# f-dangel/vivit

Measured on AMD Instinct MI355X. Metric: GGN eigenpairs/sec (Gram build + symeig), MLP 784-512-10, batch=4096, higher is better.
Workload: dtype f32

## Files before the change

### vivit_amd/csrc/common.h

```cpp
#pragma once
#include <hip/hip_runtime.h>
#include <stddef.h>
#include <stdint.h>

#include "../../include/vivit_hip.h"

namespace vivit {

typedef float f32x16 __attribute__((ext_vector_type(16)));
typedef float f32x4 __attribute__((ext_vector_type(4)));

static inline int64_t cdiv(int64_t a, int64_t b) { return (a + b - 1) / b; }
static inline size_t align_up(size_t x, size_t a) { return (x + a - 1) / a * a; }

static inline int launch_status() {
  return hipGetLastError() == hipSuccess ? VIVIT_OK : VIVIT_E_LAUNCH;
}

static inline bool ensure_dynamic_lds(const void *fn, int bytes, unsigned long long &done) {
  int dev = 0;
  if (hipGetDevice(&dev) != hipSuccess) return false;
  const unsigned long long bit = 1ull << (dev & 63);
  if (done & bit) return true;
  if (hipFuncSetAttribute(fn, hipFuncAttributeMaxDynamicSharedMemorySize, bytes) != hipSuccess) return false;
  return true;
}

enum { LAY_K = 0, LAY_M = 1 };

struct GemmDesc {
  const float *A;
  const float *B;
  float *C;
  int64_t M, N, K, lda, ldb, ldc;
};

struct GemmArgs {
  const float *A;
  const float *B;
  float *C;
  int64_t M, N, K, lda, ldb, ldc;
  float alpha, beta;
  int ksplit;
  int64_t kchunk;
  float *slab;
  int tiles_m, tiles_n;
  int syrk;
  int a_vec, b_vec;
  const GemmDesc *desc;
  int sbw;
  const int *gate = nullptr;
  int gate_mask = 0;
};

int gemm_launch(int alay, int blay, const float *A, const float *B, float *C, int64_t M, int64_t N,
                int64_t K, int64_t lda, int64_t ldb, int64_t ldc, float alpha, float beta, bool syrk,
                void *workspace, size_t workspace_bytes, hipStream_t stream);
size_t gemm_workspace_bytes(int64_t M, int64_t N, int64_t K, bool syrk);
int gemm_lower_launch(const float *A, const float *B, float *C, int64_t n, int64_t K, int64_t lda, int64_t ldb,
                      int64_t ldc, float alpha, float beta, hipStream_t stream);
int gemm_batched_launch(int alay, int blay, const GemmDesc *desc, int batch, int64_t maxM, int64_t maxN, float alpha,
                        float beta, hipStream_t stream);

bool skinny_applicable(int64_t M, int64_t N, int64_t K);
size_t skinny_workspace_bytes(int64_t K, int64_t n, int64_t P);
int skinny_nn_launch(const float *coef, int64_t ldc_, const float *V, int64_t ldv, float *out, int64_t ldo, int64_t K,
                     int64_t n, int64_t P, float alpha, float beta, void *ws, size_t ws_bytes, hipStream_t stream);

bool prof_enabled();
int prof_stride();
void prof_begin(int kind, double work, hipStream_t stream);
void prof_end(int kind, hipStream_t stream);
enum { PROF_STAGE_BEGIN = 0, PROF_STAGE_PREP = 1, PROF_STAGE_SY2SB = 2, PROF_STAGE_SB2ST = 3, PROF_STAGE_TRIDIAG = 4,
       PROF_STAGE_Q2 = 5, PROF_STAGE_Q1 = 6, PROF_STAGE_OUTPUT = 7, PROF_STAGE_SYTRD = 8,
       PROF_STAGE_SY2SB_PP = 9, PROF_STAGE_SY2SB_UPD = 10, PROF_NUM_STAGES = 11 };
void prof_mark(int stage, hipStream_t stream);

int *persist_timeout_word(hipStream_t stream);
int persist_override();
int persist_fault();

inline int device_cu_count() {
  static int cached[64] = {0};
  int dev = 0;
  if (hipGetDevice(&dev) != hipSuccess) return 0;
  int &c = cached[dev & 63];
  if (c == 0) {
    int v = 0;
    if (hipDeviceGetAttribute(&v, hipDeviceAttributeMultiprocessorCount, dev) != hipSuccess) v = -1;
    c = v > 0 ? v : -1;
  }
  return c;
}

}
```

### vivit_amd/csrc/gemm64.hip

```cpp
#include "gemm_plan.h"

namespace vivit {

constexpr int G64_NST = 7;
constexpr int G64_TA = 64 * BK, G64_TB = 256 * BK, G64_STG = G64_TA + G64_TB;
constexpr int GEMM64_LDS_BYTES = G64_NST * G64_STG * 4;

template <int ALAY, int BLAY>
__global__ __launch_bounds__(256, 1) void gemm64_dma_kernel(GemmArgs p) {
  extern __shared__ __attribute__((aligned(16))) float smem3[];
  if (p.gate && (*p.gate & p.gate_mask) == 0) return;
  const int tj = blockIdx.x;
  const int tid = threadIdx.x, lane = tid & 63, wave = tid >> 6;
  const int r = lane & 31, h = lane >> 5;
  const int64_t col0 = (int64_t)tj * 256;
  const int64_t kbeg = (int64_t)blockIdx.y * p.kchunk;
  const int64_t kend = (kbeg + p.kchunk < p.K) ? kbeg + p.kchunk : p.K;
  const int nt = (int)((kend - kbeg) / BK);

  f32x16 acc[2][2];
  auto clear_acc = [&]() __attribute__((always_inline)) {
#pragma unroll
    for (int i = 0; i < 2; ++i)
#pragma unroll
// ... 324 lines not shown
static bool gemm64_attrs() {
  static unsigned long long attr_done = 0;
  int dev = 0;
  if (hipGetDevice(&dev) != hipSuccess) return false;
  if (attr_done & (1ull << (dev & 63))) return true;
  const struct { const void *fn; int bytes; } kernels[] = {
      {reinterpret_cast<const void *>(gemm64_dma_kernel<LAY_K, LAY_K>), GEMM64_LDS_BYTES},
      {reinterpret_cast<const void *>(gemm64_dma_kernel<LAY_K, LAY_M>), GEMM64_LDS_BYTES},
      {reinterpret_cast<const void *>(gemm64_dma_kernel<LAY_M, LAY_K>), GEMM64_LDS_BYTES},
      {reinterpret_cast<const void *>(gemm64_dma_kernel<LAY_M, LAY_M>), GEMM64_LDS_BYTES},
      {reinterpret_cast<const void *>(gemm64_bx_kernel<LAY_K>), GEMM64X_LDS_BYTES},
      {reinterpret_cast<const void *>(gemm64_bx_kernel<LAY_M>), GEMM64X_LDS_BYTES},
      {reinterpret_cast<const void *>(gemm64_bx_kernel<LAY_K, true>), GEMM64X_LDS_BYTES},
      {reinterpret_cast<const void *>(gemm64_bx_kernel<LAY_M, true>), GEMM64X_LDS_BYTES}};
  for (const auto &k : kernels)
    if (!ensure_dynamic_lds(k.fn, k.bytes, attr_done)) return false;
  attr_done |= 1ull << (dev & 63);
  return true;
}

bool plan_gemm64(const GemmShape &sh, GemmPlan &pl) {
  const int64_t M = sh.M, N = sh.N, K = sh.K;
  if (sh.syrk || !(M <= 64 && N >= 2048 && K >= 2048 && (K % BK) == 0)) return false;
  pl = GemmPlan{};
  pl.route = GemmRoute::Gemm64;
  const int64_t tiles = cdiv(N, 256), ktiles = K / BK;
  int64_t s = 1;
  double best = 0.0;
  for (int64_t c = 1; c <= 24; ++c) {
    if (c > 1 && ktiles / c < 64) break;
    const int64_t wgs = tiles * c;
    const double fill = (double)wgs / (double)(256 * cdiv(wgs, 256));
    const double score = wgs >= 512 ? fill : fill * 0.5 * (double)wgs / 512.0;
    if (score > best + 1e-9) { best = score; s = c; }
  }
  pl.kchunk = cdiv(ktiles, s) * BK;
  pl.ksplit = (int)cdiv(K, pl.kchunk);
  const bool strict = gemm64_bx_enabled() && sh.pub;
  pl.slab_bytes = (pl.ksplit > 1 || strict) ? (size_t)pl.ksplit * (size_t)M * (size_t)N * sizeof(float) : 0;
  pl.bytes = pl.slab_bytes;
  if (!gemm64_bx_enabled()) return true;
  pl.a_off = align_up(pl.slab_bytes, 256);
  const size_t pieces_end = pl.a_off + (size_t)ktiles * 6144;
  pl.flags_off = align_up(pieces_end, 256);
  pl.bytes = strict ? pl.flags_off + 256 : pieces_end;
  return true;
}

static bool gemm64_bx_reach(int blay, int64_t ldb) {
  return (int64_t)(blay == LAY_K ? 255 : 15) * ldb * 4 + 1024 < ((int64_t)1 << 32);
}

int launch_gemm64(const GemmPlan &pl, const GemmShape &sh, int alay, int blay, GemmArgs p, void *workspace, size_t workspace_bytes,
                         hipStream_t stream) {
  p.ksplit = pl.ksplit;
  p.kchunk = pl.kchunk;
  const bool bx = gemm64_bx_enabled() && gemm64_bx_reach(blay, p.ldb);
  const bool strict = bx && sh.pub;
  p.slab = nullptr;
  if (p.ksplit > 1 || strict) {
    if (!workspace || workspace_bytes < pl.slab_bytes) return VIVIT_E_WORKSPACE;
    p.slab = ws_at<float>(workspace, pl.slab_off);
  }
  uint4 *apieces = nullptr;
  int *flag = nullptr;
  if (bx) {
    if (!workspace || workspace_bytes < pl.bytes) return VIVIT_E_WORKSPACE;
    apieces = ws_at<uint4>(workspace, pl.a_off);
    if (strict) flag = ws_at<int>(workspace, pl.flags_off);
  }
  if (!gemm64_attrs()) return VIVIT_E_LAUNCH;
  if (flag && hipMemsetAsync(flag, 0, sizeof(int), stream) != hipSuccess) return VIVIT_E_LAUNCH;
  p.tiles_m = 1;
  p.tiles_n = (int)cdiv(p.N, 256);
  p.syrk = 0;
  p.desc = nullptr;
  dim3 grid((unsigned)p.tiles_n, (unsigned)p.ksplit, 1);
  auto launch_dma = [&](const GemmArgs &q) {
    with_layouts(alay, blay, [&](auto LA, auto LB) { gemm64_dma_kernel<LA, LB><<<grid, 256, GEMM64_LDS_BYTES, stream>>>(q); });
  };
  const unsigned kt = (unsigned)(p.K / BK);
  if (strict) {
    with_layout(alay, [&](auto L) { g64_split_a_kernel<L, true><<<kt, 128, 0, stream>>>(p.A, p.lda, p.M, apieces, flag); });
    with_layout(blay, [&](auto L) { gemm64_bx_kernel<L, true><<<grid, 256, GEMM64X_LDS_BYTES, stream>>>(p, apieces, flag); });
    int st = launch_status();
    if (st != VIVIT_OK) return st;
    GemmArgs f = p;
    f.gate = flag;
    f.gate_mask = tls_bx_gate_mask;
    launch_dma(f);
  } else if (bx) {
    with_layout(alay, [&](auto L) { g64_split_a_kernel<L><<<kt, 128, 0, stream>>>(p.A, p.lda, p.M, apieces, nullptr); });
    with_layout(blay, [&](auto L) { gemm64_bx_kernel<L><<<grid, 256, GEMM64X_LDS_BYTES, stream>>>(p, apieces, nullptr); });
  } else {
    launch_dma(p);
  }
  int st = launch_status();
  if (st != VIVIT_OK) return st;
  if (p.slab) {
    launch_gemm_reduce(p.slab, p.C, p.M, p.N, p.ldc, p.ksplit, p.alpha, p.beta, 0, stream);
    st = launch_status();
  }
  return st;
}

}
```

### vivit_amd/csrc/gemm_f32.hip

```cpp
#include "gemm_plan.h"

namespace vivit {

__global__ __launch_bounds__(256) void gemm_reduce_kernel(const float *__restrict__ slab, float *__restrict__ C,
                                                          int64_t M, int64_t N, int64_t ldc, int ksplit,
                                                          float alpha, float beta, int syrk, int tile = BM) {
  const int64_t idx = (int64_t)blockIdx.x * 256 + threadIdx.x;
  if (idx >= M * N) return;
  const int64_t i = idx / N, j = idx - i * N;
  int64_t src = idx;
  if (syrk && (j / tile) > (i / tile)) src = j * N + i;
  float s = 0.f;
  for (int z = 0; z < ksplit; ++z) s += slab[(int64_t)z * M * N + src];
  float v = alpha * s;
  if (beta != 0.f) v += beta * C[i * ldc + j];
  C[i * ldc + j] = v;
}
void launch_gemm_reduce(const float *slab, float *C, int64_t M, int64_t N, int64_t ldc, int ksplit, float alpha, float beta, int syrk,
                        hipStream_t stream, int tile) {
  gemm_reduce_kernel<<<(unsigned)cdiv(M * N, 256), 256, 0, stream>>>(slab, C, M, N, ldc, ksplit, alpha, beta, syrk, tile);
}

__global__ __launch_bounds__(256) void scale_c_kernel(float *__restrict__ C, int64_t M, int64_t N, int64_t ldc, float beta) {
  const int64_t idx = (int64_t)blockIdx.x * 256 + threadIdx.x;
  if (idx >= M * N) return;
  const int64_t i = idx / N, j = idx - i * N;
  C[i * ldc + j] = beta == 0.f ? 0.f : beta * C[i * ldc + j];
}
void launch_scale_c(float *C, int64_t M, int64_t N, int64_t ldc, float beta, hipStream_t stream) {
  scale_c_kernel<<<(unsigned)cdiv(M * N, 256), 256, 0, stream>>>(C, M, N, ldc, beta);
}

size_t gemm_workspace_bytes(int64_t M, int64_t N, int64_t K, bool syrk) {
  if (M <= 0 || N <= 0 || K <= 0) return 0;
  const GemmShape sh{M, N, K, syrk, syrk, bx_public_product()};
  GemmShape whole = sh;
  whole.K = K / BK * BK;
  size_t b = 0;
  GemmPlan pl;
  if (plan_tile256_bx(whole, pl) && pl.bytes > b) b = pl.bytes;
  if (plan_tile256(whole, pl) && pl.bytes > b) b = pl.bytes;
  if (plan_bx_splitk(whole, pl) && pl.bytes > b) b = pl.bytes;
  if (plan_gemm64(whole, pl) && pl.bytes > b) b = pl.bytes;
  if (plan_tsk(sh, pl) && pl.bytes > b) b = pl.bytes;
  if (plan_tile128(sh, pl) && pl.bytes > b) b = pl.bytes;
  return b;
}

int gemm_launch(int alay, int blay, const float *A, const float *B, float *C, int64_t M, int64_t N,
                int64_t K, int64_t lda, int64_t ldb, int64_t ldc, float alpha, float beta, bool syrk,
                void *workspace, size_t workspace_bytes, hipStream_t stream) {
  if (M < 0 || N < 0 || K < 0) return VIVIT_E_BADARG;
  if (M == 0 || N == 0) return VIVIT_OK;
  if (!C || ldc < N) return VIVIT_E_BADARG;
  if (K == 0) {
    launch_scale_c(C, M, N, ldc, beta, stream);
    return launch_status();
  }
  if (!A || !B) return VIVIT_E_BADARG;
  if (lda < (alay == LAY_K ? K : M) || ldb < (blay == LAY_K ? K : N)) return VIVIT_E_BADARG;
  if (syrk && (M != N || alay != blay)) return VIVIT_E_BADARG;

  GemmArgs p;
  p.A = A; p.B = B; p.C = C;
  p.M = M; p.N = N; p.K = K; p.lda = lda; p.ldb = ldb; p.ldc = ldc;
  p.alpha = alpha; p.beta = beta;
  const GemmShape sh{M, N, K, syrk, A == B && lda == ldb && M == N && alay == blay, bx_public_product()};
  const bool ptr_vec = operand_vec(A, lda) && operand_vec(B, ldb);
  const auto holds = [&](const GemmPlan &q) { return workspace && workspace_bytes >= q.bytes; };
  GemmPlan pl;
  if (ptr_vec && (alay == LAY_K || (M & 3) == 0) && (blay == LAY_K || (N & 3) == 0)) {
    GemmShape whole = sh;
    whole.K = p.K = K / BK * BK;
    bool on256 = true;
    int st = VIVIT_OK;
    if (plan_tile256_bx(whole, pl) && holds(pl)) {
      st = launch_tile256_bx(pl, whole, alay, blay, p, workspace, stream);
    } else if (plan_tile256(whole, pl)) {
      if (pl.ksplit > 1 && !holds(pl)) {
        const size_t fit = workspace ? workspace_bytes / ((size_t)M * (size_t)N * sizeof(float)) : 1;
        plan_tile256(whole, pl, fit < 1 ? 1 : (int)(fit < 4 ? fit : 4));
      }
      st = launch_tile256(pl, whole, alay, blay, p, workspace, stream);
    } else if (plan_bx_splitk(whole, pl) && holds(pl)) {
      st = launch_bx_splitk(pl, whole, alay, blay, p, workspace, stream);
    } else {
      on256 = false;
      p.K = K;
    }
    if (on256) {
      if (st != VIVIT_OK || whole.K == K) return st;
      const float *At = A + (alay == LAY_K ? whole.K : whole.K * lda), *Bt = B + (blay == LAY_K ? whole.K : whole.K * ldb);
      return gemm_launch(alay, blay, At, Bt, C, M, N, K - whole.K, lda, ldb, ldc, alpha, 1.f, syrk, workspace, workspace_bytes, stream);
    }
  }
  if (gemm64_enabled() && ptr_vec && (alay == LAY_K || ((M & 3) == 0 && M >= 4)) && (blay == LAY_K || ((N & 3) == 0 && N >= 4)) &&
      plan_gemm64(sh, pl))
    return launch_gemm64(pl, sh, alay, blay, p, workspace, workspace_bytes, stream);
  if (tsk_enabled() && ptr_vec && alay == LAY_K && blay == LAY_K && plan_tsk(sh, pl))
    return launch_tsk(pl, p, workspace, workspace_bytes, stream);
  plan_tile128(sh, pl);
  return launch_tile128(pl, sh, alay, blay, p, workspace, workspace_bytes, stream);
}

template <bool VEC>
__global__ __launch_bounds__(256) void syrk_diag_kernel(const float *__restrict__ A, int64_t K, int64_t lda, const float *__restrict__ G,
                                                        int64_t ldg, float alpha, float beta, float *__restrict__ dout) {
  __shared__ double red[4];
  const int tid = threadIdx.x;
  const int64_t row = blockIdx.x;
  const float *a = A + row * lda;
  double acc[4] = {0.0, 0.0, 0.0, 0.0};
  if constexpr (VEC) {
    const int64_t K4 = K / 4;
    int64_t c = tid;
    for (; c + 3 * 256 < K4; c += 4 * 256) {
      float4 v[4];
#pragma unroll
      for (int u = 0; u < 4; ++u) v[u] = *reinterpret_cast<const float4 *>(a + 4 * (c + 256 * u));
#pragma unroll
      for (int u = 0; u < 4; ++u) {
        acc[0] = fma((double)v[u].x, (double)v[u].x, acc[0]);
        acc[1] = fma((double)v[u].y, (double)v[u].y, acc[1]);
        acc[2] = fma((double)v[u].z, (double)v[u].z, acc[2]);
        acc[3] = fma((double)v[u].w, (double)v[u].w, acc[3]);
      }
    }
    for (; c < K4; c += 256) {
      const float4 v = *reinterpret_cast<const float4 *>(a + 4 * c);
      acc[0] = fma((double)v.x, (double)v.x, acc[0]);
      acc[1] = fma((double)v.y, (double)v.y, acc[1]);
      acc[2] = fma((double)v.z, (double)v.z, acc[2]);
      acc[3] = fma((double)v.w, (double)v.w, acc[3]);
    }
    for (int64_t k = 4 * K4 + tid; k < K; k += 256) acc[0] = fma((double)a[k], (double)a[k], acc[0]);
  } else {
    for (int64_t k = tid; k < K; k += 256) acc[k & 3] = fma((double)a[k], (double)a[k], acc[k & 3]);
  }
  double sum = (acc[0] + acc[1]) + (acc[2] + acc[3]);
#pragma unroll
  for (int off = 32; off > 0; off >>= 1) sum += __shfl_xor(sum, off, 64);
  if ((tid & 63) == 0) red[tid >> 6] = sum;
  __syncthreads();
  if (tid == 0) {
    const double tot = (red[0] + red[1]) + (red[2] + red[3]);
    const double old = beta != 0.f ? (double)beta * (double)G[row * ldg + row] : 0.0;
    dout[row] = (float)(old + (double)alpha * tot);
  }
}

__global__ __launch_bounds__(256) void syrk_diag_store_kernel(float *__restrict__ G, int64_t ldg, int64_t n, const float *__restrict__ d) {
// ... 80 lines not shown
```

### vivit_amd/csrc/gemm_plan.h

```cpp
#pragma once
#include <cstdlib>

#include "gemm_tile.h"

namespace vivit {

enum class GemmRoute { Tile256Bx, Tile256, BxSplitK, Gemm64, Tsk, Tile128 };

struct GemmShape {
  int64_t M, N, K;
  bool syrk;
  bool same;
  bool pub;
};

struct GemmPlan {
  GemmRoute route;
  int ksplit;
  int64_t kchunk;
  int kt_split;
  size_t slab_off, slab_bytes;
  size_t a_off, b_off;
  size_t flags_off;
  size_t bytes;
// ... 10 lines not shown
  else if (alay == LAY_K && blay == LAY_M) f(K{}, M{});
  else if (alay == LAY_M && blay == LAY_K) f(M{}, K{});
  else f(M{}, M{});
}
template <class F>
static void with_layout(int lay, F &&f) {
  if (lay == LAY_K) f(std::integral_constant<int, LAY_K>{});
  else f(std::integral_constant<int, LAY_M>{});
}

static int operand_vec(const float *X, int64_t ld) { return ((reinterpret_cast<uintptr_t>(X) & 15) == 0 && (ld & 3) == 0) ? 1 : 0; }

static int64_t tile_grid(int64_t tiles_m, int64_t tiles_n, bool syrk, int *sbw) {
  const int w = syrk ? 16 : sb_width((int)tiles_m, (int)tiles_n), h = 256 / w;
  *sbw = w;
  const int64_t sbm = cdiv(tiles_m, h), sbn = cdiv(tiles_n, w);
  const int64_t nsb = syrk ? sbm * (sbm + 1) / 2 : sbm * sbn;
  return nsb * 256 > 0x7fffffffLL ? -1 : nsb;
}

static int env_int(const char *name, int dflt) {
  const char *e = getenv(name);
  return e ? atoi(e) : dflt;
}
inline bool gemm256_enabled() { static const int v = env_int("VIVIT_GEMM256", -1); return v != 0; }
inline bool bx_splitk_enabled() { static const int v = env_int("VIVIT_GEMM_BXSPLITK", -1); return v != 0; }
inline bool gemm64_enabled() { static const int v = env_int("VIVIT_GEMM64", -1); return v != 0; }
inline bool tsk_enabled() { static const int v = env_int("VIVIT_GEMM_TSK", -1); return v != 0; }
inline int gemm_split_mode() {
  static const int v = env_int("VIVIT_GEMM_SPLIT", 6);
  return (v == 0 || v == 3 || v == 6 || v == 9) ? v : 6;
}
inline bool bx_asm_enabled() { static const int v = env_int("VIVIT_BX_ASM", 1); return v != 0; }
inline bool gemm64_bx_enabled() { static const int v = env_int("VIVIT_GEMM64_BX", 1); return v != 0 && gemm_split_mode() != 0; }

constexpr int BX_GATE_RANGE = 1, BX_GATE_TINY = 2;
inline thread_local int tls_bx_gate_mask = BX_GATE_RANGE;
inline bool bx_public_product() { return (tls_bx_gate_mask & BX_GATE_TINY) != 0; }

struct BxStrictScope {
  int saved;
  BxStrictScope() : saved(tls_bx_gate_mask) { tls_bx_gate_mask = BX_GATE_RANGE | BX_GATE_TINY; }
  ~BxStrictScope() { tls_bx_gate_mask = saved; }
};

bool plan_tile256_bx(const GemmShape &sh, GemmPlan &pl);
int launch_tile256_bx(const GemmPlan &pl, const GemmShape &sh, int alay, int blay, GemmArgs p, void *workspace, hipStream_t stream);
bool plan_tile256(const GemmShape &sh, GemmPlan &pl, int max_split = 4);
int launch_tile256(const GemmPlan &pl, const GemmShape &sh, int alay, int blay, GemmArgs p, void *workspace, hipStream_t stream);
bool plan_bx_splitk(const GemmShape &sh, GemmPlan &pl);
int launch_bx_splitk(const GemmPlan &pl, const GemmShape &sh, int alay, int blay, GemmArgs p, void *workspace, hipStream_t stream);
bool plan_gemm64(const GemmShape &sh, GemmPlan &pl);
int launch_gemm64(const GemmPlan &pl, const GemmShape &sh, int alay, int blay, GemmArgs p, void *workspace, size_t workspace_bytes,
                  hipStream_t stream);
bool plan_tsk(const GemmShape &sh, GemmPlan &pl);
int launch_tsk(const GemmPlan &pl, const GemmArgs &g, void *workspace, size_t workspace_bytes, hipStream_t stream);
bool plan_tile128(const GemmShape &sh, GemmPlan &pl);
int launch_tile128(const GemmPlan &pl, const GemmShape &sh, int alay, int blay, GemmArgs p, void *workspace, size_t workspace_bytes,
                   hipStream_t stream);

int launch_fp32_standin(int alay, int blay, GemmArgs f, dim3 grid, const int *flag, hipStream_t stream);
bool tile256_attrs();

void launch_gemm_reduce(const float *slab, float *C, int64_t M, int64_t N, int64_t ldc, int ksplit, float alpha, float beta, int syrk,
                        hipStream_t stream, int tile = BM);
void launch_scale_c(float *C, int64_t M, int64_t N, int64_t ldc, float beta, hipStream_t stream);

}
```

### vivit_amd/csrc/sy2sb.hip

```cpp
#include <cstdlib>

#include "common.h"
#include "device_utils.h"
#include "eig_internal.h"

namespace vivit {

constexpr int SNB = 64;
constexpr int QT = 128;
constexpr int SGRP = 8;

__global__ __launch_bounds__(256) void sb_panel_load_kernel(const float *__restrict__ A, int64_t lda, int64_t j0, int64_t mp,
                                                            float *__restrict__ pan) {
  const int64_t idx = (int64_t)blockIdx.x * 256 + threadIdx.x;
  if (idx >= mp * SNB) return;
  const int64_t r = idx / SNB, c = idx - r * SNB;
  pan[idx] = A[(j0 + SNB + r) * lda + j0 + c];
}

__global__ __launch_bounds__(256) void sb_panel_load_row_kernel(const float *__restrict__ A, int64_t lda, int64_t j0, int64_t mp,
                                                                float *__restrict__ pan) {
  __shared__ float t[SNB][SNB + 1];
  const int64_t r0 = (int64_t)blockIdx.x * SNB;
  const int tid = threadIdx.x;
  for (int idx = tid; idx < SNB * SNB; idx += 256) {
    const int c = idx / SNB, rr = idx % SNB;
    t[c][rr] = r0 + rr < mp ? A[(j0 + c) * lda + j0 + SNB + r0 + rr] : 0.f;
  }
  __syncthreads();
  for (int idx = tid; idx < SNB * SNB; idx += 256) {
    const int rr = idx / SNB, c = idx % SNB;
    if (r0 + rr < mp) pan[(r0 + rr) * SNB + c] = t[c][rr];
  }
}

__global__ __launch_bounds__(256) void coef_gather_kernel(const float *__restrict__ S, int64_t lds_, int64_t g, int kp,
                                                          float *__restrict__ Coef) {
  const int idx = blockIdx.x * 256 + threadIdx.x;
  if (idx >= SNB * kp) return;
  const int k = idx / SNB, m = idx % SNB;
  Coef[(int64_t)m * kp + k] = S[(int64_t)k * lds_ + g + m];
}


__global__ __launch_bounds__(256) void qr_step_kernel(float *__restrict__ pan, int64_t mp, int c, int ncol, int nwg, QrPart pt,
                                                      float *__restrict__ vdst1, float *__restrict__ vdst2, int64_t lds_, int64_t gi0,
                                                      float *__restrict__ A, int64_t lda, int64_t j0,
                                                      float *__restrict__ tau1, float *__restrict__ betas) {
  __shared__ float tile[QT][SNB + 1];
  __shared__ float vs[QT], xs2[QT];
  __shared__ float zs[SNB];
  __shared__ float zq[4][SNB];
  __shared__ __attribute__((aligned(16))) float zq16[16][SNB];
  const int tid = threadIdx.x;
  const int64_t r0 = (int64_t)blockIdx.x * QT;
  constexpr int NTL = QT * (SNB / 4) / 256;
  float4 tl[NTL];
#pragma unroll
  for (int i = 0; i < NTL; ++i) {
    const int idx = tid + 256 * i;
    const int rl = idx / (SNB / 4), c4 = (idx - rl * (SNB / 4)) * 4;
    const int64_t r = r0 + rl;
    tl[i] = *reinterpret_cast<const float4 *>(pan + (r < mp ? r : 0) * SNB + c4);
  }
  const int par = c & 1;
  const float *uin = pt.u + (int64_t)par * nwg * SNB;
  const float *din = pt.diag + par * SNB;
  const int cq4 = tid & 15, q16 = tid >> 4;
  float4 pv[20];
#pragma unroll
  for (int i = 0; i < 20; ++i) {
    const int w = q16 + 16 * i;
    pv[i] = *reinterpret_cast<const float4 *>(uin + (int64_t)(w < nwg ? w : 0) * SNB + 4 * cq4);
  }
  const float din_c = din[c >= 0 ? c : 0], din_t = din[tid & (SNB - 1)];
  __builtin_amdgcn_sched_barrier(0);
#pragma unroll
  for (int i = 0; i < NTL; ++i) {
    const int idx = tid + 256 * i;
    const int rl = idx / (SNB / 4), c4 = (idx - rl * (SNB / 4)) * 4;
    const bool ok = r0 + rl < mp;
    tile[rl][c4 + 0] = ok ? tl[i].x : 0.f;
    tile[rl][c4 + 1] = ok ? tl[i].y : 0.f;
    tile[rl][c4 + 2] = ok ? tl[i].z : 0.f;
    tile[rl][c4 + 3] = ok ? tl[i].w : 0.f;
  }
  if (c >= 0) {
    {
      float4 acc = make_float4(0.f, 0.f, 0.f, 0.f);
#pragma unroll
      for (int i = 0; i < 20; ++i)
        if (q16 + 16 * i < nwg) { acc.x += pv[i].x; acc.y += pv[i].y; acc.z += pv[i].z; acc.w += pv[i].w; }
      for (int w0 = q16 + 16 * 20; w0 < nwg; w0 += 16 * 20) {
        float4 v[20];
// ... 256 lines not shown
      float *dst = pan + r * SNB + 8 * cg;
      *reinterpret_cast<float4 *>(dst) = make_float4(x[0][0], x[0][1], x[0][2], x[0][3]);
      *reinterpret_cast<float4 *>(dst + 4) = make_float4(x[0][4], x[0][5], x[0][6], x[0][7]);
    }
    if (tid == 0 && s_flag[1]) {
      betas[0] = __builtin_nanf("");
      __hip_atomic_fetch_or(pw.tmo, PERSIST_TMO_PANEL_QR, __ATOMIC_RELAXED, __HIP_MEMORY_SCOPE_AGENT);
    }
  }
}

static bool qr_persist_enabled() {
  static int on = -1;
  if (on < 0) {
    const char *e = getenv("VIVIT_QR_PERSIST");
    on = e ? atoi(e) : 1;
  }
  return on != 0 && persist_override() != 0;
}
constexpr size_t QR_PERSIST_WS_BYTES = sizeof(float) * (2 * QP_WG * SNB + 2 * SNB) + 64 * sizeof(int) + 256;

static bool qr_persist_launch(float *pan, int64_t mp, int ncol, void *wsp, float *v1, float *v2, int64_t ldn, int64_t gi0, float *A,
                              int64_t lda, int64_t j0, float *tau1, float *betas, hipStream_t stream) {
  if (!qr_persist_enabled() || mp > (int64_t)QP_WG * 64 * 20 || device_cu_count() < 256) return false;
  QrPersistWs pw;
  pw.ubuf = reinterpret_cast<float *>(align_up(reinterpret_cast<uintptr_t>(wsp), 256));
  pw.dbuf = pw.ubuf + 2 * QP_WG * SNB;
  pw.counter = reinterpret_cast<int *>(pw.dbuf + 2 * SNB);
  pw.tmo = persist_timeout_word(stream);
  pw.fault = persist_fault();
  if (!pw.tmo) return false;
  if (hipMemsetAsync(pw.counter, 0, 64 * sizeof(int), stream) != hipSuccess) return false;
  const int64_t ri = cdiv(mp, (int64_t)QP_WG * 64);
  const dim3 grid(8 * QP_WG);
#define QP_LAUNCH(RI) qr_persist_kernel<RI><<<grid, QP_THREADS, 0, stream>>>(pan, mp, ncol, pw, v1, v2, ldn, gi0, A, lda, j0, tau1, betas)
  for (int attempt = 0; attempt < 2; ++attempt) {
    pw.attempt = attempt;
    if (ri <= 1) QP_LAUNCH(1);
    else if (ri <= 2) QP_LAUNCH(2);
    else if (ri <= 3) QP_LAUNCH(3);
    else if (ri <= 5) QP_LAUNCH(5);
    else if (ri <= 8) QP_LAUNCH(8);
    else if (ri <= 12) QP_LAUNCH(12);
    else if (ri <= 16) QP_LAUNCH(16);
    else QP_LAUNCH(20);
  }
#undef QP_LAUNCH
  return true;
}

struct Sk64Args {
  const float *Coef;
  const float *B;
  float *Out;
  int64_t ldcoef, ldb, ldo, N;
  int K;
  float alpha, beta;
};
constexpr int SK_LDC = 36, SK_COLS = 128, SK_LDB = SK_COLS + 4, SK_NT = SK_COLS / 64;

__global__ __launch_bounds__(256) void skinny64_kernel(Sk64Args p) {
  __shared__ __attribute__((aligned(16))) float sC[64 * SK_LDC];
  __shared__ __attribute__((aligned(16))) float sB[32 * SK_LDB];
  const int tid = threadIdx.x, lane = tid & 63, wave = tid >> 6;
  const int r = lane & 31, h = lane >> 5, wm = wave >> 1, wn = wave & 1;
  const int64_t c0 = (int64_t)blockIdx.x * SK_COLS;
  f32x16 acc[SK_NT];
#pragma unroll
  for (int t = 0; t < SK_NT; ++t)
#pragma unroll
    for (int e = 0; e < 16; ++e) acc[t][e] = 0.f;
  constexpr int NLB = 32 * SK_COLS / 4 / 256;
  float4 rc[2], rb[NLB];
  auto gload = [&](int k0) __attribute__((always_inline)) {
#pragma unroll
    for (int i = 0; i < 2; ++i) {
      const int idx = tid + 256 * i;
      const int m = idx >> 3, kq = (idx & 7) * 4;
      rc[i] = *reinterpret_cast<const float4 *>(p.Coef + (int64_t)m * p.ldcoef + k0 + kq);
    }
#pragma unroll
    for (int i = 0; i < NLB; ++i) {
      const int idx = tid + 256 * i;
      const int kr = idx / (SK_COLS / 4), cq = (idx % (SK_COLS / 4)) * 4;
      const int64_t c = c0 + cq;
      rb[i] = *reinterpret_cast<const float4 *>(p.B + (int64_t)(k0 + kr) * p.ldb + (c < p.N ? c : 0));
    }
    __builtin_amdgcn_sched_barrier(0);
  };
  gload(0);
  for (int k0 = 0; k0 < p.K; k0 += 32) {
    __syncthreads();
#pragma unroll
    for (int i = 0; i < 2; ++i) {
      const int idx = tid + 256 * i;
      *reinterpret_cast<float4 *>(sC + (idx >> 3) * SK_LDC + (idx & 7) * 4) = rc[i];
    }
#pragma unroll
    for (int i = 0; i < NLB; ++i) {
      const int idx = tid + 256 * i;
      const int kr = idx / (SK_COLS / 4), cq = (idx % (SK_COLS / 4)) * 4;
      *reinterpret_cast<float4 *>(sB + kr * SK_LDB + cq) = c0 + cq < p.N ? rb[i] : make_float4(0.f, 0.f, 0.f, 0.f);
    }
    __syncthreads();
    if (k0 + 32 < p.K) gload(k0 + 32);
    const float *pa = sC + (32 * wm + r) * SK_LDC + 4 * h;
#pragma unroll
    for (int j = 0; j < 4; ++j) {
      const float4 a4 = *reinterpret_cast<const float4 *>(pa + 8 * j);
      const float av[4] = {a4.x, a4.y, a4.z, a4.w};
      float bv[4][SK_NT];
#pragma unroll
      for (int i = 0; i < 4; ++i)
#pragma unroll
        for (int t = 0; t < SK_NT; ++t) bv[i][t] = sB[(8 * j + 4 * h + i) * SK_LDB + 64 * wn + 32 * t + r];
#pragma unroll
      for (int i = 0; i < 4; ++i)
#pragma unroll
        for (int t = 0; t < SK_NT; ++t) acc[t] = __builtin_amdgcn_mfma_f32_32x32x2f32(av[i], bv[i][t], acc[t], 0, 0, 0);
    }
  }
#pragma unroll
  for (int t = 0; t < SK_NT; ++t) {
    const int64_t c = c0 + 64 * wn + 32 * t + r;
    if (c < p.N) {
#pragma unroll
      for (int e = 0; e < 16; ++e) {
        const int m = 32 * wm + (e & 3) + 8 * (e >> 2) + 4 * h;
        float *o = p.Out + (int64_t)m * p.ldo + c;
        float v = p.alpha * acc[t][e];
        if (p.beta != 0.f) v += p.beta * *o;
        *o = v;
      }
    }
  }
}

static bool skinny64_launch(const float *Coef, int64_t ldcoef, const float *B, int64_t ldb, float *Out, int64_t ldo, int64_t N, int64_t K,
                            float alpha, float beta, hipStream_t stream) {
  if (K < 32 || K % 32 != 0 || K > 4096 || N % 4 != 0 || ldb % 4 != 0 || ldcoef % 4 != 0 ||
      (reinterpret_cast<uintptr_t>(Coef) & 15) || (reinterpret_cast<uintptr_t>(B) & 15))
    return false;
  Sk64Args a;
  a.Coef = Coef; a.B = B; a.Out = Out; a.ldcoef = ldcoef; a.ldb = ldb; a.ldo = ldo; a.N = N; a.K = (int)K; a.alpha = alpha; a.beta = beta;
  skinny64_kernel<<<(unsigned)cdiv(N, SK_COLS), 256, 0, stream>>>(a);
  return true;
}

__global__ __launch_bounds__(256) void w_coef_kernel(const float *__restrict__ T, const float *__restrict__ G, float *__restrict__ Coef) {
  __shared__ float sT[SNB][SNB + 1], sG[SNB][SNB + 1], sU[SNB][SNB + 1];
  const int tid = threadIdx.x, lane = tid & 63, wave = tid >> 6;
  const int r = lane & 31, h = lane >> 5, qi = (wave >> 1) * 32, qj = (wave & 1) * 32;
  for (int idx = tid; idx < SNB * SNB; idx += 256) {
    sT[idx / SNB][idx % SNB] = T[idx];
    sG[idx / SNB][idx % SNB] = G[idx];
  }
  __syncthreads();
  f32x16 acc;
#pragma unroll
  for (int e = 0; e < 16; ++e) acc[e] = 0.f;
#pragma unroll 8
  for (int s2 = 0; s2 < SNB / 2; ++s2) acc = __builtin_amdgcn_mfma_f32_32x32x2f32(sT[2 * s2 + h][qi + r], sG[2 * s2 + h][qj + r], acc, 0, 0, 0);
#pragma unroll
  for (int e = 0; e < 16; ++e) sU[qi + (e & 3) + 8 * (e >> 2) + 4 * h][qj + r] = acc[e];
  __syncthreads();
#pragma unroll
  for (int e = 0; e < 16; ++e) acc[e] = 0.f;
#pragma unroll 8
  for (int s2 = 0; s2 < SNB / 2; ++s2) acc = __builtin_amdgcn_mfma_f32_32x32x2f32(sU[qi + r][2 * s2 + h], sT[2 * s2 + h][qj + r], acc, 0, 0, 0);
#pragma unroll
  for (int e = 0; e < 16; ++e) {
    const int a_ = qi + (e & 3) + 8 * (e >> 2) + 4 * h, b_ = qj + r;
    Coef[a_ * 2 * SNB + b_] = -0.5f * acc[e];
    Coef[a_ * 2 * SNB + SNB + b_] = sT[b_][a_];
  }
}

__global__ __launch_bounds__(256) void sb_panel_store_kernel(float *__restrict__ A, int64_t lda, int64_t j0, int64_t mp,
                                                             const float *__restrict__ pan, const float *__restrict__ betas) {
  const int idx = blockIdx.x * 256 + threadIdx.x;
  if (idx >= SNB * SNB) return;
  const int r = idx / SNB, c = idx - r * SNB;
  if (r >= mp) return;
  A[(j0 + SNB + r) * lda + j0 + c] = (r < c) ? pan[(int64_t)r * SNB + c] : (r == c ? betas[c] : 0.f);
}

__global__ __launch_bounds__(256) void larft_kernel(const float *__restrict__ S, int64_t lds_, const float *__restrict__ tau, int nb,
                                                    int nvalid, float *__restrict__ T) {
  constexpr int H = SNB / 2, LD = SNB + 1;
  __shared__ float Ss[SNB * LD], Ts[SNB * LD], Xs[H * (H + 1)], taus[SNB];
  const int tid = threadIdx.x;
  for (int idx = tid; idx < SNB * SNB; idx += 256) {
    Ss[(idx / SNB) * LD + (idx % SNB)] = S[(int64_t)(idx / SNB) * lds_ + (idx % SNB)];
    Ts[(idx / SNB) * LD + (idx % SNB)] = 0.f;
  }
  if (tid < SNB) taus[tid] = (tid < nvalid && tid < nb) ? tau[tid] : 0.f;
  __syncthreads();
// ... 58 lines not shown
    const int64_t q = mp < n ? mp : n;
    size_t a = gemm_workspace_bytes(SNB, SNB, q, false);
    size_t b = gemm_workspace_bytes(SNB, q, q, false);
    size_t c = gemm_workspace_bytes(SNB, q, SNB, false);
    size_t d = 0, e = 0, f = 0;
    for (int g = 1; g < SGRP; ++g) {
      const size_t d1 = gemm_workspace_bytes(SNB, 2 * SNB * g + SNB, q, false), e1 = gemm_workspace_bytes(SNB, q, 2 * SNB * g, false);
      const size_t f1 = gemm_workspace_bytes(q, SNB, 2 * SNB * g, false);
      d = d1 > d ? d1 : d; e = e1 > e ? e1 : e; f = f1 > f ? f1 : f;
    }
    m = a > m ? a : m; m = b > m ? b : m; m = c > m ? c : m;
    m = d > m ? d : m; m = e > m ? e : m; m = f > m ? f : m;
    const size_t u = gemm_workspace_bytes(q, q, (int64_t)2 * SNB * SGRP, true);
    m = u > m ? u : m;
  }
  size_t a = gemm_workspace_bytes(SNB, SNB, n, false), b = gemm_workspace_bytes(SNB, n, n, false);
  m = a > m ? a : m; m = b > m ? b : m;
  return m * 2;
}

Sy2sbWs sy2sb_layout(Arena &a, int64_t n) {
  const int64_t nwg = cdiv(n, QT) + 1;
  Sy2sbWs ws;
  ws.pan = a.take<float>(n * SNB);
  ws.stackA = a.take<float>(2 * SGRP * SNB * n);
  ws.stackB = a.take<float>(2 * SGRP * SNB * n);
  ws.xt = a.take<float>(SNB * n);
  ws.G12 = a.take<float>(SNB * 2 * SNB * SGRP);
  ws.qp.u = a.take<float>(2 * nwg * SNB);
  ws.qp.diag = a.take<float>(2 * SNB);
  ws.qpw = a.take<char>(QR_PERSIST_WS_BYTES);
  ws.S = a.take<float>(SNB * SNB);
  ws.T = a.take<float>(SNB * SNB);
  ws.Y3 = a.take<float>(SNB * SNB);
  ws.S2 = a.take<float>(SNB * SNB);
  ws.tau1 = a.take<float>(n);
  ws.betas = a.take<float>(SNB);
  ws.gws_bytes = sy2sb_gemm_ws_bytes(n);
  ws.gws = a.take<char>(ws.gws_bytes);
  return ws;
}

size_t sy2sb_workspace_bytes(int64_t n) {
  Arena m;
  sy2sb_layout(m, n);
  return m.used() + 1024;
}

int sy2sb_launch(float *A, int64_t n, int64_t lda, const Sy2sbWs &ws, hipStream_t stream) {
  if (hipMemsetAsync(ws.tau1, 0, sizeof(float) * n, stream) != hipSuccess) return VIVIT_E_LAUNCH;

  const int64_t ldn = n;
  const bool rowmode = (n % 4 == 0) && (lda % 4 == 0) && (reinterpret_cast<uintptr_t>(A) & 15) == 0;
  auto factor_panel = [&](int64_t j0, float *v1, float *v2) -> int {
    const int64_t mp = n - j0 - SNB, gi0 = j0 + SNB;
    const int ncol = (int)(mp < SNB ? mp : SNB);
    const int g = (int)cdiv(mp, QT);
    if (rowmode) sb_panel_load_row_kernel<<<(unsigned)cdiv(mp, SNB), 256, 0, stream>>>(A, lda, j0, mp, ws.pan);
    else sb_panel_load_kernel<<<(unsigned)cdiv(mp * SNB, 256), 256, 0, stream>>>(A, lda, j0, mp, ws.pan);
    if (!qr_persist_launch(ws.pan, mp, ncol, ws.qpw, v1, v2, ldn, gi0, A, lda, j0, ws.tau1, ws.betas, stream))
      for (int c = -1; c < ncol; ++c)
        qr_step_kernel<<<g, 256, 0, stream>>>(ws.pan, mp, c, ncol, g, ws.qp, v1, v2, ldn, gi0, A, lda, j0, ws.tau1, ws.betas);
    sb_panel_store_kernel<<<(unsigned)cdiv(SNB * SNB, 256), 256, 0, stream>>>(A, lda, j0, mp, ws.pan, ws.betas);
    return launch_status();
  };
  auto compute_w = [&](int64_t j0, float *Vt, float *Wt, float *Wcopy, int64_t kp, const float *sAg, const float *sBg) -> int {
    const int64_t mp = n - j0 - SNB, gi0 = j0 + SNB;
    const int ncol = (int)(mp < SNB ? mp : SNB);
    float *A22 = A + gi0 * lda + gi0;
    int st;
    prof_mark(PROF_STAGE_SY2SB, stream);
    st = gemm_launch(LAY_K, LAY_M, Vt, A22, Wt, SNB, mp, mp, ldn, lda, ldn, 1.f, 0.f, false, ws.gws, ws.gws_bytes, stream);
    prof_mark(PROF_STAGE_SY2SB_PP, stream);
    if (st != VIVIT_OK) return st;
    const int64_t ldg = kp + SNB;
    st = gemm_launch(LAY_K, LAY_K, Vt, sAg, ws.G12, SNB, ldg, mp, ldn, ldn, ldg, 1.f, 0.f, false, ws.gws, ws.gws_bytes, stream);
    if (st != VIVIT_OK) return st;
    larft_kernel<<<1, 256, 0, stream>>>(ws.G12 + kp, ldg, ws.tau1 + j0, SNB, ncol, ws.T);
    if (kp > 0) {
      if (!skinny64_launch(ws.G12, ldg, sBg, ldn, Wt, ldn, mp, kp, -1.f, 1.f, stream)) {
        st = gemm_launch(LAY_K, LAY_M, ws.G12, sBg, Wt, SNB, mp, kp, ldg, ldn, ldn, -1.f, 1.f, false, ws.gws, ws.gws_bytes, stream);
        if (st != VIVIT_OK) return st;
      }
    }
    st = gemm_launch(LAY_K, LAY_K, Wt, Vt, ws.S2, SNB, SNB, mp, ldn, ldn, SNB, 1.f, 0.f, false, ws.gws, ws.gws_bytes, stream);
    if (st != VIVIT_OK) return st;
    w_coef_kernel<<<1, 256, 0, stream>>>(ws.T, ws.S2, ws.G12);
    if (Wt == Vt + (int64_t)SNB * ldn &&
        skinny64_launch(ws.G12, 2 * SNB, Vt, ldn, Wcopy, ldn, mp, 2 * SNB, 1.f, 0.f, stream))
      return hipMemcpy2DAsync(Wt, sizeof(float) * ldn, Wcopy, sizeof(float) * ldn, sizeof(float) * mp, SNB, hipMemcpyDeviceToDevice,
                              stream) == hipSuccess ? VIVIT_OK : VIVIT_E_LAUNCH;
    float *Xt = ws.xt + gi0;
    st = gemm_launch(LAY_M, LAY_M, ws.T, Wt, Xt, SNB, mp, SNB, SNB, ldn, ldn, 1.f, 0.f, false, ws.gws, ws.gws_bytes, stream);
    if (st != VIVIT_OK) return st;
    if (hipMemcpy2DAsync(Wt, sizeof(float) * ldn, Xt, sizeof(float) * ldn, sizeof(float) * mp, SNB, hipMemcpyDeviceToDevice,
                         stream) != hipSuccess)
      return VIVIT_E_LAUNCH;
    st = gemm_launch(LAY_K, LAY_M, ws.G12, Vt, Wt, SNB, mp, SNB, 2 * SNB, ldn, ldn, 1.f, 1.f, false, ws.gws, ws.gws_bytes, stream);
    if (st != VIVIT_OK) return st;
    return hipMemcpy2DAsync(Wcopy, sizeof(float) * ldn, Wt, sizeof(float) * ldn, sizeof(float) * mp, SNB, hipMemcpyDeviceToDevice,
                            stream) == hipSuccess ? VIVIT_OK : VIVIT_E_LAUNCH;
  };

  float *sA = ws.stackA, *sB = ws.stackB;
  for (int64_t j0 = 0; j0 + SNB < n;) {
    int st;
    if (hipMemsetAsync(sA, 0, sizeof(float) * 2 * SGRP * SNB * n, stream) != hipSuccess) return VIVIT_E_LAUNCH;
    if (hipMemsetAsync(sB, 0, sizeof(float) * 2 * SGRP * SNB * n, stream) != hipSuccess) return VIVIT_E_LAUNCH;
    int np = 0;
    int64_t gi_last = 0;
    for (; np < SGRP && j0 + SNB < n; ++np, j0 += SNB) {
      const int64_t gi = j0 + SNB;
      const int64_t kp = (int64_t)2 * SNB * np;
      if (np > 0) {
        const int64_t gc = gi - SNB;
        bool done = false;
        if (rowmode) {
          coef_gather_kernel<<<(unsigned)cdiv(SNB * kp, 256), 256, 0, stream>>>(sA, ldn, gc, (int)kp, ws.G12);
          done = skinny64_launch(ws.G12, kp, sB + gc, ldn, A + gc * lda + gc, lda, n - gc, kp, -1.f, 1.f, stream);
        }
        if (!done) {
          if (rowmode) return VIVIT_E_UNSUPPORTED;
          st = gemm_launch(LAY_M, LAY_M, sA + gc, sB + gc, A + gc * lda + gc, n - gc, SNB, kp, ldn, ldn, lda, -1.f, 1.f, false,
                           ws.gws, ws.gws_bytes, stream);
          if (st != VIVIT_OK) return st;
        }
      }
      float *Vrow = sA + kp * n, *Wrow = sA + (kp + SNB) * n;
      st = factor_panel(j0, Vrow, sB + (kp + SNB) * n);
      if (st != VIVIT_OK) return st;
      st = compute_w(j0, Vrow + gi, Wrow + gi, sB + kp * n + gi, kp, sA + gi, sB + gi);
      if (st != VIVIT_OK) return st;
      gi_last = gi;
    }
    const int64_t mt = n - gi_last;
    prof_mark(PROF_STAGE_SY2SB, stream);
    st = gemm_launch(LAY_M, LAY_M, sA + gi_last, sB + gi_last, A + gi_last * lda + gi_last, mt, mt, (int64_t)2 * SNB * np, ldn, ldn,
                     lda, -1.f, 1.f, true, ws.gws, ws.gws_bytes, stream);
    prof_mark(PROF_STAGE_SY2SB_UPD, stream);
    if (st != VIVIT_OK) return st;
  }
  return launch_status();
}

struct PanelQrWs {
  QrPart qp;
  float *S;
  void *qpw, *gws;
  size_t gws_bytes;
};

static PanelQrWs panel_qr_layout(Arena &a, int64_t mp) {
  const int64_t nwg = cdiv(mp, QT) + 1;
  PanelQrWs ws;
  ws.qp.u = a.take<float>(2 * nwg * SNB);
  ws.qp.diag = a.take<float>(2 * SNB);
  ws.S = a.take<float>(SNB * SNB);
  ws.qpw = a.take<char>(QR_PERSIST_WS_BYTES);
  ws.gws_bytes = gemm_workspace_bytes(SNB, SNB, mp, false);
  ws.gws = a.take<char>(ws.gws_bytes);
  return ws;
}

size_t sy2sb_panel_qr_workspace_bytes(int64_t mp) {
  Arena m;
  panel_qr_layout(m, mp);
  return m.used() + 1024;
}

int sy2sb_panel_qr_launch(float *pan, int64_t mp, float *Vt, int64_t ldv, float *tau, float *betas, float *T, void *wsbase,
                          size_t ws_bytes, hipStream_t stream) {
  if (ws_bytes < sy2sb_panel_qr_workspace_bytes(mp)) return VIVIT_E_WORKSPACE;
  Arena a(wsbase, ws_bytes);
  const PanelQrWs ws = panel_qr_layout(a, mp);
  if (a.overflow()) return VIVIT_E_WORKSPACE;
  const QrPart qp = ws.qp;
  float *S = ws.S;
  void *qpw = ws.qpw, *gws = ws.gws;
  const size_t gws_bytes = ws.gws_bytes;
  const int ncol = (int)(mp < SNB ? mp : SNB);
  const int g = (int)cdiv(mp, QT);
  if (hipMemsetAsync(tau, 0, sizeof(float) * SNB, stream) != hipSuccess) return VIVIT_E_LAUNCH;
// ... 51 lines not shown
```

Baseline: 7416.

## Fuse split-K reduce, coef gather, panel load and copy into skinny64 kernel

Extends the skinny64 kernel so it can read a transposed coefficient matrix directly, dropping the coef_gather kernel. Its epilogue can also write the panel buffer, which skips the panel load kernel, and write a second output, which replaces a 2D memcpy. A GEMM's split-K reduction can now be deferred and folded into the following skinny64 epilogue. To support this, the workspace is split in halves so the deferred slab is not overwritten by the intervening GEMM. The goal is fewer small kernel launches and memory passes in the sy2sb band reduction, at the cost of more complex epilogues and strided slab reads.

Result: no change. 7431, median of 3 (+0.2%).

```diff
diff --git a/vivit_amd/csrc/common.h b/vivit_amd/csrc/common.h
--- a/vivit_amd/csrc/common.h
+++ b/vivit_amd/csrc/common.h
@@ -53,9 +53,14 @@
   int gate_mask = 0;
 };
 
+struct GemmDeferred {
+  const float *slab = nullptr;
+  int ksplit = 0;
+};
+
 int gemm_launch(int alay, int blay, const float *A, const float *B, float *C, int64_t M, int64_t N,
                 int64_t K, int64_t lda, int64_t ldb, int64_t ldc, float alpha, float beta, bool syrk,
-                void *workspace, size_t workspace_bytes, hipStream_t stream);
+                void *workspace, size_t workspace_bytes, hipStream_t stream, GemmDeferred *defer = nullptr);
 size_t gemm_workspace_bytes(int64_t M, int64_t N, int64_t K, bool syrk);
 int gemm_lower_launch(const float *A, const float *B, float *C, int64_t n, int64_t K, int64_t lda, int64_t ldb,
                       int64_t ldc, float alpha, float beta, hipStream_t stream);
diff --git a/vivit_amd/csrc/gemm64.hip b/vivit_amd/csrc/gemm64.hip
--- a/vivit_amd/csrc/gemm64.hip
+++ b/vivit_amd/csrc/gemm64.hip
@@ -400,7 +400,7 @@
 }
 
 int launch_gemm64(const GemmPlan &pl, const GemmShape &sh, int alay, int blay, GemmArgs p, void *workspace, size_t workspace_bytes,
-                         hipStream_t stream) {
+                         hipStream_t stream, GemmDeferred *defer) {
   p.ksplit = pl.ksplit;
   p.kchunk = pl.kchunk;
   const bool bx = gemm64_bx_enabled() && gemm64_bx_reach(blay, p.ldb);
@@ -445,7 +445,10 @@
   }
   int st = launch_status();
   if (st != VIVIT_OK) return st;
-  if (p.slab) {
+  if (p.slab && defer && !strict && p.ksplit > 1) {
+    defer->slab = p.slab;
+    defer->ksplit = p.ksplit;
+  } else if (p.slab) {
     launch_gemm_reduce(p.slab, p.C, p.M, p.N, p.ldc, p.ksplit, p.alpha, p.beta, 0, stream);
     st = launch_status();
   }
diff --git a/vivit_amd/csrc/gemm_f32.hip b/vivit_amd/csrc/gemm_f32.hip
--- a/vivit_amd/csrc/gemm_f32.hip
+++ b/vivit_amd/csrc/gemm_f32.hip
@@ -49,7 +49,8 @@
 
 int gemm_launch(int alay, int blay, const float *A, const float *B, float *C, int64_t M, int64_t N,
                 int64_t K, int64_t lda, int64_t ldb, int64_t ldc, float alpha, float beta, bool syrk,
-                void *workspace, size_t workspace_bytes, hipStream_t stream) {
+                void *workspace, size_t workspace_bytes, hipStream_t stream, GemmDeferred *defer) {
+  if (defer) *defer = GemmDeferred{};
   if (M < 0 || N < 0 || K < 0) return VIVIT_E_BADARG;
   if (M == 0 || N == 0) return VIVIT_OK;
   if (!C || ldc < N) return VIVIT_E_BADARG;
@@ -96,7 +97,7 @@
   }
   if (gemm64_enabled() && ptr_vec && (alay == LAY_K || ((M & 3) == 0 && M >= 4)) && (blay == LAY_K || ((N & 3) == 0 && N >= 4)) &&
       plan_gemm64(sh, pl))
-    return launch_gemm64(pl, sh, alay, blay, p, workspace, workspace_bytes, stream);
+    return launch_gemm64(pl, sh, alay, blay, p, workspace, workspace_bytes, stream, (alpha == 1.f && beta == 0.f) ? defer : nullptr);
   if (tsk_enabled() && ptr_vec && alay == LAY_K && blay == LAY_K && plan_tsk(sh, pl))
     return launch_tsk(pl, p, workspace, workspace_bytes, stream);
   plan_tile128(sh, pl);
diff --git a/vivit_amd/csrc/gemm_plan.h b/vivit_amd/csrc/gemm_plan.h
--- a/vivit_amd/csrc/gemm_plan.h
+++ b/vivit_amd/csrc/gemm_plan.h
@@ -86,7 +86,7 @@
 int launch_bx_splitk(const GemmPlan &pl, const GemmShape &sh, int alay, int blay, GemmArgs p, void *workspace, hipStream_t stream);
 bool plan_gemm64(const GemmShape &sh, GemmPlan &pl);
 int launch_gemm64(const GemmPlan &pl, const GemmShape &sh, int alay, int blay, GemmArgs p, void *workspace, size_t workspace_bytes,
-                  hipStream_t stream);
+                  hipStream_t stream, GemmDeferred *defer = nullptr);
 bool plan_tsk(const GemmShape &sh, GemmPlan &pl);
 int launch_tsk(const GemmPlan &pl, const GemmArgs &g, void *workspace, size_t workspace_bytes, hipStream_t stream);
 bool plan_tile128(const GemmShape &sh, GemmPlan &pl);
diff --git a/vivit_amd/csrc/sy2sb.hip b/vivit_amd/csrc/sy2sb.hip
--- a/vivit_amd/csrc/sy2sb.hip
+++ b/vivit_amd/csrc/sy2sb.hip
@@ -32,14 +32,6 @@
     const int rr = idx / SNB, c = idx % SNB;
     if (r0 + rr < mp) pan[(r0 + rr) * SNB + c] = t[c][rr];
   }
-}
-
-__global__ __launch_bounds__(256) void coef_gather_kernel(const float *__restrict__ S, int64_t lds_, int64_t g, int kp,
-                                                          float *__restrict__ Coef) {
-  const int idx = blockIdx.x * 256 + threadIdx.x;
-  if (idx >= SNB * kp) return;
-  const int k = idx / SNB, m = idx % SNB;
-  Coef[(int64_t)m * kp + k] = S[(int64_t)k * lds_ + g + m];
 }
 
 
@@ -402,9 +394,10 @@
 struct Sk64Args {
   const float *Coef;
   const float *B;
-  float *Out;
+  float *Out, *Out2, *pan;
+  const float *slab;
   int64_t ldcoef, ldb, ldo, N;
-  int K;
+  int K, coef_t, nsplit;
   float alpha, beta;
 };
 constexpr int SK_LDC = 36, SK_COLS = 128, SK_LDB = SK_COLS + 4, SK_NT = SK_COLS / 64;
@@ -426,8 +419,13 @@
 #pragma unroll
     for (int i = 0; i < 2; ++i) {
       const int idx = tid + 256 * i;
-      const int m = idx >> 3, kq = (idx & 7) * 4;
-      rc[i] = *reinterpret_cast<const float4 *>(p.Coef + (int64_t)m * p.ldcoef + k0 + kq);
+      if (p.coef_t) {
+        const int kr = idx >> 4, mq = (idx & 15) * 4;
+        rc[i] = *reinterpret_cast<const float4 *>(p.Coef + (int64_t)(k0 + kr) * p.ldcoef + mq);
+      } else {
+        const int m = idx >> 3, kq = (idx & 7) * 4;
+        rc[i] = *reinterpret_cast<const float4 *>(p.Coef + (int64_t)m * p.ldcoef + k0 + kq);
+      }
     }
 #pragma unroll
     for (int i = 0; i < NLB; ++i) {
@@ -444,7 +442,15 @@
 #pragma unroll
     for (int i = 0; i < 2; ++i) {
       const int idx = tid + 256 * i;
-      *reinterpret_cast<float4 *>(sC + (idx >> 3) * SK_LDC + (idx & 7) * 4) = rc[i];
+      if (p.coef_t) {
+        const int kr = idx >> 4, mq = (idx & 15) * 4;
+        sC[(mq + 0) * SK_LDC + kr] = rc[i].x;
+        sC[(mq + 1) * SK_LDC + kr] = rc[i].y;
+        sC[(mq + 2) * SK_LDC + kr] = rc[i].z;
+        sC[(mq + 3) * SK_LDC + kr] = rc[i].w;
+      } else {
+        *reinterpret_cast<float4 *>(sC + (idx >> 3) * SK_LDC + (idx & 7) * 4) = rc[i];
+      }
     }
 #pragma unroll
     for (int i = 0; i < NLB; ++i) {
@@ -474,25 +480,53 @@
   for (int t = 0; t < SK_NT; ++t) {
     const int64_t c = c0 + 64 * wn + 32 * t + r;
     if (c < p.N) {
+      float old[16];
+      if (p.slab) {
+        const int64_t MN = (int64_t)64 * p.N;
+#pragma unroll
+        for (int e = 0; e < 16; ++e) old[e] = 0.f;
+        for (int z = 0; z < p.nsplit; ++z) {
+          const float *sz = p.slab + (int64_t)z * MN + c;
+#pragma unroll
+          for (int e = 0; e < 16; ++e) old[e] += sz[(int64_t)(32 * wm + (e & 3) + 8 * (e >> 2) + 4 * h) * p.N];
+        }
+      }
+      float res[16];
 #pragma unroll
       for (int e = 0; e < 16; ++e) {
         const int m = 32 * wm + (e & 3) + 8 * (e >> 2) + 4 * h;
         float *o = p.Out + (int64_t)m * p.ldo + c;
         float v = p.alpha * acc[t][e];
-        if (p.beta != 0.f) v += p.beta * *o;
+        if (p.beta != 0.f) v += p.beta * (p.slab ? old[e] : *o);
         *o = v;
-      }
-    }
-  }
-}
-
+        if (p.Out2) p.Out2[(int64_t)m * p.ldo + c] = v;
+        res[e] = v;
+      }
+      if (p.pan && c >= SNB) {
+        float *pr = p.pan + (c - SNB) * SNB + 32 * wm + 4 * h;
+#pragma unroll
+        for (int q = 0; q < 4; ++q)
+          *reinterpret_cast<float4 *>(pr + 8 * q) = make_float4(res[4 * q], res[4 * q + 1], res[4 * q + 2], res[4 * q + 3]);
+      }
+    }
+  }
+}
+
+struct Sk64Fuse {
+  bool coef_t = false;
+  float *Out2 = nullptr;
+  float *pan = nullptr;
+  const float *slab = nullptr;
+  int nsplit = 0;
+};
 static bool skinny64_launch(const float *Coef, int64_t ldcoef, const float *B, int64_t ldb, float *Out, int64_t ldo, int64_t N, int64_t K,
-                            float alpha, float beta, hipStream_t stream) {
+                            float alpha, float beta, hipStream_t stream, const Sk64Fuse &f = Sk64Fuse{}) {
   if (K < 32 || K % 32 != 0 || K > 4096 || N % 4 != 0 || ldb % 4 != 0 || ldcoef % 4 != 0 ||
-      (reinterpret_cast<uintptr_t>(Coef) & 15) || (reinterpret_cast<uintptr_t>(B) & 15))
+      (reinterpret_cast<uintptr_t>(Coef) & 15) || (reinterpret_cast<uintptr_t>(B) & 15) || (reinterpret_cast<uintptr_t>(f.pan) & 15))
     return false;
   Sk64Args a;
   a.Coef = Coef; a.B = B; a.Out = Out; a.ldcoef = ldcoef; a.ldb = ldb; a.ldo = ldo; a.N = N; a.K = (int)K; a.alpha = alpha; a.beta = beta;
+  a.coef_t = f.coef_t ? 1 : 0; a.Out2 = f.Out2; a.pan = f.pan; a.slab = f.slab; a.nsplit = f.nsplit;
   skinny64_kernel<<<(unsigned)cdiv(N, SK_COLS), 256, 0, stream>>>(a);
   return true;
 }
@@ -657,12 +691,14 @@
 
   const int64_t ldn = n;
   const bool rowmode = (n % 4 == 0) && (lda % 4 == 0) && (reinterpret_cast<uintptr_t>(A) & 15) == 0;
-  auto factor_panel = [&](int64_t j0, float *v1, float *v2) -> int {
+  auto factor_panel = [&](int64_t j0, float *v1, float *v2, bool pan_ready) -> int {
     const int64_t mp = n - j0 - SNB, gi0 = j0 + SNB;
     const int ncol = (int)(mp < SNB ? mp : SNB);
     const int g = (int)cdiv(mp, QT);
-    if (rowmode) sb_panel_load_row_kernel<<<(unsigned)cdiv(mp, SNB), 256, 0, stream>>>(A, lda, j0, mp, ws.pan);
-    else sb_panel_load_kernel<<<(unsigned)cdiv(mp * SNB, 256), 256, 0, stream>>>(A, lda, j0, mp, ws.pan);
+    if (!pan_ready) {
+      if (rowmode) sb_panel_load_row_kernel<<<(unsigned)cdiv(mp, SNB), 256, 0, stream>>>(A, lda, j0, mp, ws.pan);
+      else sb_panel_load_kernel<<<(unsigned)cdiv(mp * SNB, 256), 256, 0, stream>>>(A, lda, j0, mp, ws.pan);
+    }
     if (!qr_persist_launch(ws.pan, mp, ncol, ws.qpw, v1, v2, ldn, gi0, A, lda, j0, ws.tau1, ws.betas, stream))
       for (int c = -1; c < ncol; ++c)
         qr_step_kernel<<<g, 256, 0, stream>>>(ws.pan, mp, c, ncol, g, ws.qp, v1, v2, ldn, gi0, A, lda, j0, ws.tau1, ws.betas);
@@ -674,16 +710,26 @@
     const int ncol = (int)(mp < SNB ? mp : SNB);
     float *A22 = A + gi0 * lda + gi0;
     int st;
+    const int64_t ldg = kp + SNB;
+    const size_t half = (ws.gws_bytes / 2) & ~(size_t)255;
+    const bool halves = rowmode && gemm_workspace_bytes(SNB, mp, mp, false) <= half && gemm_workspace_bytes(SNB, ldg, mp, false) <= half;
+    void *gws_g = halves ? static_cast<char *>(ws.gws) + half : ws.gws;
+    const size_t gws_bytes = halves ? half : ws.gws_bytes;
+    GemmDeferred pt;
     prof_mark(PROF_STAGE_SY2SB, stream);
-    st = gemm_launch(LAY_K, LAY_M, Vt, A22, Wt, SNB, mp, mp, ldn, lda, ldn, 1.f, 0.f, false, ws.gws, ws.gws_bytes, stream);
+    st = gemm_launch(LAY_K, LAY_M, Vt, A22, Wt, SNB, mp, mp, ldn, lda, ldn, 1.f, 0.f, false, ws.gws, gws_bytes, stream,
+                     (halves && kp > 0) ? &pt : nullptr);
     prof_mark(PROF_STAGE_SY2SB_PP, stream);
     if (st != VIVIT_OK) return st;
-    const int64_t ldg = kp + SNB;
-    st = gemm_launch(LAY_K, LAY_K, Vt, sAg, ws.G12, SNB, ldg, mp, ldn, ldn, ldg, 1.f, 0.f, false, ws.gws, ws.gws_bytes, stream);
+    st = gemm_launch(LAY_K, LAY_K, Vt, sAg, ws.G12, SNB, ldg, mp, ldn, ldn, ldg, 1.f, 0.f, false, gws_g, gws_bytes, stream);
     if (st != VIVIT_OK) return st;
     larft_kernel<<<1, 256, 0, stream>>>(ws.G12 + kp, ldg, ws.tau1 + j0, SNB, ncol, ws.T);
     if (kp > 0) {
-      if (!skinny64_launch(ws.G12, ldg, sBg, ldn, Wt, ldn, mp, kp, -1.f, 1.f, stream)) {
+      Sk64Fuse f;
+      f.slab = pt.slab;
+      f.nsplit = pt.ksplit;
+      if (!skinny64_launch(ws.G12, ldg, sBg, ldn, Wt, ldn, mp, kp, -1.f, 1.f, stream, f)) {
+        if (pt.slab) return VIVIT_E_UNSUPPORTED;
         st = gemm_launch(LAY_K, LAY_M, ws.G12, sBg, Wt, SNB, mp, kp, ldg, ldn, ldn, -1.f, 1.f, false, ws.gws, ws.gws_bytes, stream);
         if (st != VIVIT_OK) return st;
       }
@@ -691,10 +737,11 @@
     st = gemm_launch(LAY_K, LAY_K, Wt, Vt, ws.S2, SNB, SNB, mp, ldn, ldn, SNB, 1.f, 0.f, false, ws.gws, ws.gws_bytes, stream);
     if (st != VIVIT_OK) return st;
     w_coef_kernel<<<1, 256, 0, stream>>>(ws.T, ws.S2, ws.G12);
-    if (Wt == Vt + (int64_t)SNB * ldn &&
-        skinny64_launch(ws.G12, 2 * SNB, Vt, ldn, Wcopy, ldn, mp, 2 * SNB, 1.f, 0.f, stream))
-      return hipMemcpy2DAsync(Wt, sizeof(float) * ldn, Wcopy, sizeof(float) * ldn, sizeof(float) * mp, SNB, hipMemcpyDeviceToDevice,
-                              stream) == hipSuccess ? VIVIT_OK : VIVIT_E_LAUNCH;
+    if (Wt == Vt + (int64_t)SNB * ldn) {
+      Sk64Fuse f;
+      f.Out2 = Wt;
+      if (skinny64_launch(ws.G12, 2 * SNB, Vt, ldn, Wcopy, ldn, mp, 2 * SNB, 1.f, 0.f, stream, f)) return launch_status();
+    }
     float *Xt = ws.xt + gi0;
     st = gemm_launch(LAY_M, LAY_M, ws.T, Wt, Xt, SNB, mp, SNB, SNB, ldn, ldn, 1.f, 0.f, false, ws.gws, ws.gws_bytes, stream);
     if (st != VIVIT_OK) return st;
@@ -721,8 +768,10 @@
         const int64_t gc = gi - SNB;
         bool done = false;
         if (rowmode) {
-          coef_gather_kernel<<<(unsigned)cdiv(SNB * kp, 256), 256, 0, stream>>>(sA, ldn, gc, (int)kp, ws.G12);
-          done = skinny64_launch(ws.G12, kp, sB + gc, ldn, A + gc * lda + gc, lda, n - gc, kp, -1.f, 1.f, stream);
+          Sk64Fuse f;
+          f.coef_t = true;
+          f.pan = ws.pan;
+          done = skinny64_launch(sA + gc, ldn, sB + gc, ldn, A + gc * lda + gc, lda, n - gc, kp, -1.f, 1.f, stream, f);
         }
         if (!done) {
           if (rowmode) return VIVIT_E_UNSUPPORTED;
@@ -732,7 +781,7 @@
         }
       }
       float *Vrow = sA + kp * n, *Wrow = sA + (kp + SNB) * n;
-      st = factor_panel(j0, Vrow, sB + (kp + SNB) * n);
+      st = factor_panel(j0, Vrow, sB + (kp + SNB) * n, rowmode && np > 0);
       if (st != VIVIT_OK) return st;
       st = compute_w(j0, Vrow + gi, Wrow + gi, sB + kp * n + gi, kp, sA + gi, sB + gi);
       if (st != VIVIT_OK) return st;
```
